# kianmcevoy/audio_analysis

Measured on AMD Instinct MI355X. Metric: IRs/sec full report (STFT+RT60bands+zplane), 48 kHz 10 s IR, higher is better.
Workload: dtype f64; 1 GPU; metrics-only full report on 256 mono synthetic IRs per GPU per step, 10 s @ 48 kHz (SURVEY.md 8d generator), H2D included: every step uploads its batch from pinned host memory (float32, 492 MB) on a copy stream under the previous step's kernels; 4 distinct batches rotate; batch_per_gpu=256, parallelism=file-sharded dp1, gather=final

## Files before the change

audio_analysis_amd/_lib.py:

```python
from __future__ import annotations

import ctypes as C
from pathlib import Path

_LIB_PATH = Path(__file__).resolve().parent / "csrc" / "libira.so"
_lib = None
ABI_VERSION = 15

c_f32p = C.c_void_p
c_i64p = C.c_void_p
c_i32p = C.c_void_p
c_f64p = C.c_void_p
vp = C.c_void_p
i32 = C.c_int32
f64 = C.c_double
f32 = C.c_float

PROTOTYPES = {
    "ira_abi_version": (i32, []),
    "ira_error_string": (C.c_char_p, [i32]),
    "ira_peak_index": (i32, [vp, vp, vp, i32, C.c_int64, vp, vp, vp]),
    "ira_edc_db": (i32, [vp, vp, vp, i32, C.c_int64, f64, f64, vp, vp, vp, vp, vp]),
    "ira_curve_fits": (i32, [vp, vp, vp, i32, i32, f32, f32, vp, C.POINTER(f64), i32, i32, C.POINTER(f64), i32, i32,
                             f64, f64, vp, vp, vp]),
# ... 18 lines not shown
    "ira_band_tile_layout": (i32, [i32, i32, C.POINTER(i32), C.POINTER(i32)]),
    "ira_wav_probe": (i32, [C.c_char_p, vp, vp, vp, vp]),
    "ira_wav_read_pcm16": (i32, [C.c_char_p, C.c_int64, C.c_int64, i32, vp]),
    "ira_wav_probe_batch": (i32, [vp, i32, i32, vp, vp, vp, vp, vp]),
    "ira_wav_read_pcm16_batch": (i32, [vp, vp, vp, vp, vp, vp, i32, i32, vp]),
    "ira_pcm16_to_channels": (i32, [vp, C.c_int64, i32, i32, vp, vp]),
    "ira_pcm16_to_channels_jobs": (i32, [vp, vp, vp, vp, vp, vp, i32, C.c_int64, vp, vp]),
    "ira_band_mask_values": (i32, [C.POINTER(f64), f64, C.c_int64, vp, vp]),
    "ira_host_pull": (i32, [vp, C.c_int64, i32, vp, i32, vp]),
    "ira_deconv_divide": (i32, [vp, vp, vp, vp, vp, i32, i32, f64, vp, vp]),
    "ira_deconv_finish": (i32, [vp, vp, vp, vp, i32, i32, i32, i32, i32, f64, vp, vp, vp]),
    "ira_order_stats": (i32, [vp, vp, vp, i32, vp, i32, vp, vp]),
    "ira_diffusion": (i32, [vp, vp, vp, i32, i32, i32, i32, i32, f64, f64, vp, vp, vp, vp]),
    "ira_diffusion_stereo": (i32, [vp, vp, vp, vp, i32, i32, i32, i32, i32, vp, vp, vp, vp]),
    "ira_spectrum_stats": (i32, [vp, vp, vp, i32, vp, f64, f64, f64, vp, vp]),
    "ira_waterfall_rel": (i32, [vp, vp, vp, i32, i32, i32, i32, f64, vp, vp, vp]),
    "ira_logbin_aggregate": (i32, [vp, vp, vp, i32, i32, i32, vp, vp, i32, vp, vp, i32, vp]),
    "ira_ar_partial_doubles": (C.c_int64, [i32, i32]),
    "ira_ar_gram": (i32, [vp, vp, vp, vp, vp, i32, i32, i32, vp, i32, vp]),
    "ira_ar_solve": (i32, [vp, vp, i32, i32, i32, f64, vp, vp, vp, i32, vp]),
    "ira_ar_minnorm": (i32, [vp, vp, i32, i32, i32, vp, vp, vp, f64, vp]),
    "ira_ar_exact_doubles": (C.c_int64, [i32, i32, i32]),
    "ira_ar_exact": (i32, [vp, vp, vp, vp, vp, i32, i32, i32, f64, vp, vp, vp, vp, vp, f64, vp]),
    "ira_ar_refine": (i32, [vp, vp, vp, vp, vp, i32, i32, i32, vp, vp, vp, vp, vp, f64, i32, i32, vp]),
    "ira_ar_fit": (i32, [vp, vp, vp, vp, vp, i32, i32, i32, f64, vp, vp, vp, vp, i32, vp]),
    "ira_poly_roots": (i32, [vp, i32, i32, f64, vp, vp, vp]),
    "ira_fir_numerator": (i32, [vp, i32, vp, vp, vp, vp, i32, i32, vp, vp]),
    "ira_onset_index": (i32, [vp, vp, vp, i32, C.c_int64, vp, vp, f64, vp, vp]),
    "ira_energy_scratch_doubles": (C.c_int64, [i32, C.c_int64, i32]),
    "ira_energy_windows": (i32, [vp, vp, vp, vp, vp, i32, C.c_int64, vp, i32, vp, vp, vp]),
# ... 72 lines not shown
```

audio_analysis_amd/analyse/frequency_response.py:

```python
from __future__ import annotations

from dataclasses import dataclass
from pathlib import Path
from typing import List, Optional, Sequence, Tuple

import numpy as np

from ..engine import get_engine
from ._common import segment_bounds, segment_bounds_batch, wav_channels


@dataclass(frozen=True)
class FrequencyResponseAnalysisSettings:
    use_mono_downmix_for_stereo: bool = False
    trim_to_peak: bool = True
    ignore_leading_seconds: float = 0.0
    analysis_duration_seconds: Optional[float] = None
    use_hann_window: bool = True
    magnitude_floor_db: float = -120.0
    f_min_hz: float = 20.0
    f_max_hz: float = 20000.0
    smoothing_log_bins: int = 0
    log_bins_per_octave: int = 96

# ... 62 lines not shown


def spectrum_segments(eng, batch, sample_rate_hz: int, settings, what: str):
    peaks = eng.peaks(batch) if settings.trim_to_peak else np.zeros(batch.count, dtype=np.int64)
    starts, lens = segment_bounds_batch(batch.length, peaks, sample_rate_hz, settings.trim_to_peak,
                                        settings.ignore_leading_seconds, settings.analysis_duration_seconds)
    if np.any(lens < 32):
        raise ValueError(f"Not enough samples after trimming/selection to analyse {what}.")
    return starts, lens


def spectrum_device(eng, batch, sample_rate_hz: int, settings, what: str, want_phase: bool = False,
                    unwrap: bool = True, degrees: bool = True):
    starts, lens = spectrum_segments(eng, batch, sample_rate_hz, settings, what)
    spec, off, packed = eng.rfft_any_packed(batch.x, batch.off + starts, lens, bool(settings.use_hann_window))
    mag, ph = eng.spectrum_mag_phase(spec, off, lens, float(settings.magnitude_floor_db), want_phase=want_phase,
                                     packed=packed)
    phase = eng.phase_unwrap(ph, off, lens, unwrap, degrees) if want_phase else None
    nyq = 0.5 * float(sample_rate_hz)
    f_lo = float(np.clip(settings.f_min_hz, 0.0, nyq))
    f_hi = float(np.clip(settings.f_max_hz, f_lo, nyq))
    steps = np.array([rfft_bin_step(int(n), sample_rate_hz) for n in lens], dtype=np.float64)
    smoothed = False
    bins_w = int(getattr(settings, "smoothing_log_bins", 0) or 0)
    if bins_w > 1:
        s_lo = float(np.clip(settings.f_min_hz, 1.0, nyq))
        s_hi = float(np.clip(settings.f_max_hz, s_lo, nyq))
        rng = [selected_bin_range(int(n) // 2 + 1, float(st), max(1.0, s_lo), max(max(1.0, s_lo), s_hi))
               for n, st in zip(lens, steps)]
        k_lo = np.array([r[0] for r in rng], dtype=np.int32)
        nsel = np.array([r[1] for r in rng], dtype=np.int32)
        if np.all(nsel > 0):
            smoothed = eng.log_smooth(mag, off, np.ones(len(rng), np.int32), k_lo, nsel, steps, bins_w,
                                      int(getattr(settings, "log_bins_per_octave", 96)), through_float32=False)
    stats = eng.spectrum_stats(mag, off, lens, steps, f_lo, f_hi, 1000.0)
    return dict(spec=spec if packed is None else None, spec_packed=spec if packed is not None else None, off=off, packed=packed, starts=starts, lens=lens, mag=mag, phase=phase, stats=stats, f_lo=f_lo,
                f_hi=f_hi, smoothed=smoothed)


def analyse_frequency_response_batch(
    channels: Sequence[np.ndarray],
    sample_rate_hz: int,
    channel_names: Sequence[str],
    settings: FrequencyResponseAnalysisSettings,
) -> List[ChannelFrequencyResponse]:
    for c in channels:
        if c.ndim != 1:
            raise ValueError("analyse_frequency_response_for_channel expects a 1D mono array.")
    eng = get_engine()
    batch = eng.upload(list(channels))
# ... 103 lines not shown
```

audio_analysis_amd/analyse/group_delay.py:

```python
from __future__ import annotations

from dataclasses import dataclass
from pathlib import Path
from typing import List, Optional, Sequence, Tuple

import numpy as np

from ..engine import get_engine
from ._common import wav_channels
from .frequency_response import rfft_bin_step


@dataclass(frozen=True)
class GroupDelayAnalysisSettings:
    use_mono_downmix_for_stereo: bool = False
    trim_to_peak: bool = True
    ignore_leading_seconds: float = 0.0
    analysis_duration_seconds: Optional[float] = None
    use_hann_window: bool = True
    fft_size: Optional[int] = None
    f_min_hz: float = 20.0
    f_max_hz: float = 20000.0
    unwrap_phase: bool = True
    smoothing_bins: int = 0
# ... 48 lines not shown
    n = batch.count
    if starts is None:
        peaks = eng.peaks(batch) if settings.trim_to_peak else np.zeros(n, dtype=np.int64)
        starts = np.empty(n, dtype=np.int64)
        lens = np.empty(n, dtype=np.int64)
        for i in range(n):
            starts[i], lens[i] = group_delay_segment(int(batch.length[i]), int(peaks[i]), sample_rate_hz, settings)
    if np.any(lens < 1):
        raise ValueError("Not enough samples after trimming/selection to analyse group delay.")
    n_fft = np.array([fft_size_for(int(v), settings) for v in lens], dtype=np.int64)
    if np.any(n_fft < 2) or np.any(n_fft > (1 << 21)):
        raise ValueError("group delay needs 2 <= fft_size <= 2097152.")
    with eng.tagged("[gd]"):
        spec, off = eng.rfft_any(batch.x, batch.off + starts, n_fft.astype(np.int32), bool(settings.use_hann_window),
                                 data_len=np.minimum(lens, n_fft).astype(np.int32), win_len=lens.astype(np.int32))
        _, ph = eng.spectrum_mag_phase(spec, off, n_fft.astype(np.int32), -400.0, want_phase=True)
        ph64 = eng.phase_unwrap(ph, off, n_fft.astype(np.int32), bool(settings.unwrap_phase), False, as_float64=True)
        steps = np.array([rfft_bin_step(int(v), sample_rate_hz) for v in n_fft], dtype=np.float64)
        gd = eng.group_delay(ph64, off, n_fft, steps, float(sample_rate_hz))
    return dict(gd=gd, off=off, n_fft=n_fft, starts=starts, lens=lens)


_MASK_CACHE: dict = {}


def mask_range(n_fft: int, sample_rate_hz: int, f_min_hz: float, f_max_hz: float) -> Tuple[int, int]:
    key = (int(n_fft), int(sample_rate_hz), float(f_min_hz), float(f_max_hz))
    if key not in _MASK_CACHE:
        freq = np.fft.rfftfreq(int(n_fft), d=1.0 / float(sample_rate_hz))
        idx = np.nonzero((freq >= float(f_min_hz)) & (freq <= float(f_max_hz)))[0]
        _MASK_CACHE[key] = (int(idx[0]), int(idx.size)) if idx.size else (0, 0)
    return _MASK_CACHE[key]
# ... 146 lines not shown
```

audio_analysis_amd/csrc/ira_spectrum.hip:

```cpp
#include <cmath>

#include "ira_fft_reg.h"
#include "ira_log.h"

namespace {

typedef ira::cplx<double> cd;
constexpr double kPi = 3.14159265358979323846;

constexpr int ATAN_TAB = 64;

__device__ __forceinline__ void build_atan_table(double* tab, int tid) {
  if (tid <= ATAN_TAB) tab[tid] = atan((double)tid * (1.0 / ATAN_TAB));
}

__device__ __forceinline__ double atan2_table(double y, double x, const double* tab) {
  const double ax = fabs(x), ay = fabs(y);
  const double mx = fmax(ax, ay), mn = fmin(ax, ay);
  if (!(ax > 1.0e-300 && ay > 1.0e-300 && ax < 1.0e300 && ay < 1.0e300)) return atan2(y, x);
  const double t = mn / mx;
  const int k = (int)(t * (double)ATAN_TAB + 0.5);
  const double t0 = (double)k * (1.0 / ATAN_TAB);
  const double r = (t - t0) / fma(t, t0, 1.0);
  const double r2 = r * r;
  double s = fma(r2, 1.0 / 9.0, -1.0 / 7.0);
  s = fma(r2, s, 0.2);
  s = fma(r2, s, -1.0 / 3.0);
  s = fma(r2, s, 1.0);
  double a = fma(r, s, tab[k]);
  if (ay > ax) a = 1.5707963267948966 - a;
  if (x < 0.0) a = kPi - a;
  return copysign(a, y);
}

__device__ __forceinline__ double unwrap_correction(double prev, double cur) {
  const double dd = cur - prev;
  const double period = 2.0 * kPi;
  double a = dd + kPi;
  double md;
  if (a >= 0.0 && a < period) md = a;
  else if (a >= period && a < 2.0 * period) md = a - period;
  else if (a < 0.0 && a > -period) md = a;
  else md = fmod(a, period);
  if (md != 0.0) {
    if (md < 0.0) md += period;
  } else {
    md = 0.0;
  }
  double ddmod = md + (-kPi);
  if (ddmod == -kPi && dd > 0.0) ddmod = kPi;
  double corr = ddmod - dd;
  if (fabs(dd) < kPi) corr = 0.0;
  return corr;
}

__global__ __launch_bounds__(256) void mag_phase_kernel(const cd* __restrict__ spec, const int64_t* __restrict__ spec_off,
                                 const int32_t* __restrict__ L, double floor_lin, float* __restrict__ mag_db,
                                 const int64_t* __restrict__ mag_off, double* __restrict__ phase,
                                 const int64_t* __restrict__ phase_off, const int32_t* __restrict__ packed) {
  __shared__ ira::LogTabEntry ltab[ira::LOGTAB_N];
  __shared__ double atab[ATAN_TAB + 1];
  ira::build_log_table(ltab, threadIdx.x);
  build_atan_table(atab, threadIdx.x);
  __syncthreads();
  const int e = blockIdx.y;
  const long long nb = (long long)L[e] / 2 + 1;
  const cd* s = spec + spec_off[e];
  float* mo = mag_db + mag_off[e];
  double* po = phase ? phase + phase_off[e] : nullptr;
  const double floor_p = floor_lin * floor_lin;
  const float floor_db32 = (float)(20.0 * log10(floor_lin));
  const bool pk = packed != nullptr && ira::uniform(packed[e]) != 0;
  const long long l = (long long)L[e] / 2;
  const long long k_first = (long long)blockIdx.x * blockDim.x + threadIdx.x, k_step = (long long)gridDim.x * blockDim.x;
  double cs = 1.0, sn = 0.0, rc = 1.0, rs = 0.0;
  if (pk) {
    sincospi(-(double)(k_first < nb ? k_first : 0) / (double)l, &sn, &cs);
    sincospi(-(double)(k_step % (2 * l)) / (double)l, &rs, &rc);
  }
  for (long long k = k_first; k < nb; k += k_step) {
    cd v;
    if (pk) {
      const cd zk = s[k == l ? 0 : k], zl = s[(k == 0 || k == l) ? 0 : l - k];
      const auto [ev, od] = ira::hermitian_parts(zk, zl);
      v = {ev.re + (cs * od.re - sn * od.im), ev.im + (cs * od.im + sn * od.re)};
      if (k == 0 || k == l) v.im = 0.0;
      const double nc = cs * rc - sn * rs;
      sn = sn * rc + cs * rs;
      cs = nc;
    } else {
      v = s[k];
    }
    const double p = v.re * v.re + v.im * v.im;
    float db;
    if (p > 1.0e-280 && p < 1.0e280 && floor_lin > 1.0e-140) {
      db = p > floor_p ? (float)(3.0102999566398120 * ira::log2_table(p, ltab)) : floor_db32;
    } else {
      const double a = hypot(v.re, v.im);
      const double m = (a != a) ? a : fmax(a, floor_lin);
      db = (float)(20.0 * log10(m));
    }
    mo[k] = db;
    if (po) po[k] = atan2_table(v.im, v.re, atab);
  }
}

constexpr int UW_THREADS = 1024;
constexpr int UW_PER = 4;
constexpr int UW_TILE = UW_THREADS * UW_PER;

__global__ __launch_bounds__(UW_THREADS) void unwrap_kernel(const double* __restrict__ phase,
                                                            const int64_t* __restrict__ phase_off,
                                                            const int32_t* __restrict__ L, int do_unwrap,
                                                            double out_scale, float* __restrict__ out,
                                                            const int64_t* __restrict__ out_off,
                                                            double* __restrict__ out64) {
  __shared__ double wave_tot[UW_THREADS / IRA_WAVE];
  __shared__ double tile_total;
  const int e = blockIdx.x;
  const long long n = (long long)L[e] / 2 + 1;
  const double* p = phase + phase_off[e];
  float* o = out ? out + out_off[e] : nullptr;
  double* o64 = out64 ? out64 + out_off[e] : nullptr;
  const int t = threadIdx.x, lane = t & 63, wave = t >> 6;
// ... 11 lines not shown
    double prev = nprev;
#pragma unroll
    for (int r = 0; r < UW_PER; ++r) v[r] = nv[r];
    if (base + UW_TILE < n) {
      const long long j0 = i0 + UW_TILE;
      nprev = (j0 - 1 < n) ? p[j0 - 1] : 0.0;
#pragma unroll
      for (int r = 0; r < UW_PER; ++r) nv[r] = (j0 + r < n) ? p[j0 + r] : 0.0;
    }
#pragma unroll
    for (int r = 0; r < UW_PER; ++r) {
      const long long i = i0 + r;
      c[r] = (do_unwrap && i >= 1 && i < n) ? unwrap_correction(prev, v[r]) : 0.0;
      prev = v[r];
    }
    c[1] += c[0]; c[2] += c[1]; c[3] += c[2];
    double incl = c[3];
#pragma unroll
    for (int o2 = 1; o2 < 64; o2 <<= 1) {
      const double dn = __shfl_up(incl, o2, 64);
      if (lane >= o2) incl += dn;
    }
    double excl = __shfl_up(incl, 1, 64);
    if (lane == 0) excl = 0.0;
    if (lane == 63) wave_tot[wave] = incl;
    __syncthreads();
    double before = 0.0;
    for (int w = 0; w < wave; ++w) before += wave_tot[w];
    const double add = carry + (before + excl);
#pragma unroll
    for (int r = 0; r < UW_PER; ++r) {
      const long long i = i0 + r;
      if (i < n) {
        const double u = v[r] + (c[r] + add);
        if (o) o[i] = (float)(u * out_scale);
        if (o64) o64[i] = u;
      }
    }
    if (t == UW_THREADS - 1) tile_total = c[3] + add;
    __syncthreads();
    carry = tile_total;
  }
}

// ... 209 lines not shown
        const long long excl = incl - c;
        if ((excl <= rem && rem < incl) || (tid == 255 && rem >= incl)) {
          remaining[r] = rem - excl;
          bucket[r] = c;
          prefix[r] = prefix[r] | ((unsigned long long)tid << shift);
        }
      }
      __syncthreads();
    }
  }
  if (tid < nranks) o[tid] = os_unkey(prefix[tid]);
}

constexpr int ST_THREADS = 1024;

__global__ __launch_bounds__(ST_THREADS) void stats_kernel(const float* __restrict__ mag_db,
                                                           const int64_t* __restrict__ mag_off,
                                                           const int32_t* __restrict__ L,
                                                           const double* __restrict__ freq_val, float f_min, float f_max,
                                                           float probe_hz, double* __restrict__ out) {
  __shared__ double red[4][ST_THREADS / IRA_WAVE];
  __shared__ unsigned long long kred[2][ST_THREADS / IRA_WAVE];
  __shared__ long long lred[ST_THREADS / IRA_WAVE];
  __shared__ double etab[ira::EXPTAB_N];
  const int e = blockIdx.x;
  const long long n = (long long)L[e] / 2 + 1;
  const float* m = mag_db + mag_off[e];
  const double val = freq_val[e];
  const int t = threadIdx.x, lane = t & 63, wave = t >> 6;
  ira::build_exp_table(etab, t);
  __syncthreads();
  double cnt = 0.0, sfl = 0.0, sl = 0.0;
  unsigned long long best = 0ull;
  unsigned long long near = ~0ull;
  long long first_in = n;
  constexpr int ST_U = 16;
  for (long long k0 = t; k0 < n; k0 += (long long)ST_THREADS * ST_U) {
    float dbv[ST_U];
#pragma unroll
    for (int u = 0; u < ST_U; ++u) {
      const long long k = k0 + (long long)ST_THREADS * u;
      dbv[u] = m[k < n ? k : n - 1];
    }
#pragma unroll
    for (int u = 0; u < ST_U; ++u) {
      const long long k = k0 + (long long)ST_THREADS * u;
      if (k >= n) continue;
      const float f = (float)((double)k * val);
      const float d = fabsf(f - probe_hz);
      const unsigned long long nk = ((unsigned long long)__float_as_uint(d) << 32) | (unsigned long long)(uint32_t)k;
      near = nk < near ? nk : near;
      if (f >= f_min && f <= f_max) {
        const float db = dbv[u];
        uint32_t uu = __float_as_uint(db);
        uu = (uu & 0x80000000u) ? ~uu : (uu | 0x80000000u);
        if (db != db) uu = 0xFFFFFFFFu;
        const unsigned long long key = ((unsigned long long)uu << 32) | (unsigned long long)(0xFFFFFFFFu - (uint32_t)k);
        best = key > best ? key : best;
        const double y = (double)db * 0.05;
        const double lin = fabs(y) < 15.0 ? ira::exp10_table(y, etab) : exp10(y);
        cnt += 1.0; sfl += (double)f * lin; sl += lin;
        first_in = k < first_in ? k : first_in;
      }
    }
  }
  cnt = ira::wave_sum(cnt); sfl = ira::wave_sum(sfl); sl = ira::wave_sum(sl);
#pragma unroll
  for (int o = 32; o > 0; o >>= 1) {
    const unsigned long long ob = __shfl_xor(best, o, 64);
    best = ob > best ? ob : best;
    const unsigned long long on = __shfl_xor(near, o, 64);
    near = on < near ? on : near;
    const long long of = __shfl_xor(first_in, o, 64);
    first_in = of < first_in ? of : first_in;
  }
  if (lane == 0) {
    red[0][wave] = cnt; red[1][wave] = sfl; red[2][wave] = sl;
    kred[0][wave] = best; kred[1][wave] = near; lred[wave] = first_in;
  }
  __syncthreads();
  if (t == 0) {
    cnt = sfl = sl = 0.0;
    for (int w = 0; w < ST_THREADS / IRA_WAVE; ++w) {
      cnt += red[0][w]; sfl += red[1][w]; sl += red[2][w];
      best = kred[0][w] > best ? kred[0][w] : best;
      near = kred[1][w] < near ? kred[1][w] : near;
      first_in = lred[w] < first_in ? lred[w] : first_in;
    }
    double* o = out + (int64_t)e * 8;
    const long long pk = (cnt > 0.0) ? (long long)(0xFFFFFFFFu - (uint32_t)(best & 0xFFFFFFFFull)) : 0;
    const long long i1k = (long long)(near & 0xFFFFFFFFull);
    o[0] = cnt;
    o[1] = (double)pk;
    o[2] = (double)(float)((double)pk * val);
    o[3] = sfl; o[4] = sl;
    o[5] = first_in < n ? (double)(float)((double)first_in * val) : 0.0;
    o[6] = (double)i1k;
    o[7] = (double)m[i1k];
  }
}

constexpr int LS_MAX = 2048;
constexpr int LS_THREADS = 256;

__device__ __forceinline__ double ls_freq(long long k, double fstep) { return (double)(float)((double)k * fstep); }

__global__ __launch_bounds__(LS_THREADS) void log_smooth_kernel(float* __restrict__ mag, const int64_t* __restrict__ off,
                                                                const int32_t* __restrict__ stride_a,
                                                                const int32_t* __restrict__ k_lo_a,
                                                                const int32_t* __restrict__ nsel_a,
                                                                const double* __restrict__ fstep_a,
                                                                const double* __restrict__ lg_lo, const double* __restrict__ lg_hi,
                                                                const int32_t* __restrict__ count_a, int window,
                                                                int through_f32) {
// ... 106 lines not shown
                                           gd_dev);
  IRA_RETURN_LAUNCH();
}

extern "C" int32_t ira_spectrum_stats(const float* mag_db_dev, const int64_t* mag_off_dev, const int32_t* L_dev,
                                      int32_t nb, const double* freq_val_dev, double f_min_hz, double f_max_hz,
                                      double probe_hz, double* out_dev, void* stream) {
  IRA_CHECK_PTR(mag_db_dev); IRA_CHECK_PTR(mag_off_dev); IRA_CHECK_PTR(L_dev); IRA_CHECK_PTR(freq_val_dev);
  IRA_CHECK_PTR(out_dev);
  if (nb <= 0) return nb == 0 ? IRA_OK : IRA_E_SIZE;
  stats_kernel<<<nb, ST_THREADS, 0, (hipStream_t)stream>>>(mag_db_dev, mag_off_dev, L_dev, freq_val_dev,
                                                           (float)f_min_hz, (float)f_max_hz, (float)probe_hz, out_dev);
  IRA_RETURN_LAUNCH();
}

extern "C" int32_t ira_order_stats(const double* values_dev, const int64_t* off_dev, const int32_t* count_dev,
                                   int32_t nseg, const int64_t* ranks_dev, int32_t nranks, double* out_dev,
                                   void* stream) {
  IRA_CHECK_PTR(values_dev); IRA_CHECK_PTR(off_dev); IRA_CHECK_PTR(count_dev); IRA_CHECK_PTR(ranks_dev);
  IRA_CHECK_PTR(out_dev);
  if (nranks < 1 || nranks > OS_MAX_RANKS) return IRA_E_SIZE;
  if (nseg <= 0) return nseg == 0 ? IRA_OK : IRA_E_SIZE;
  order_stats_kernel<<<nseg, OS_THREADS, 0, (hipStream_t)stream>>>(values_dev, off_dev, count_dev, ranks_dev, nranks,
                                                                    out_dev);
  IRA_RETURN_LAUNCH();
}

extern "C" int32_t ira_log_smooth_db(float* mag_dev, const int64_t* off_dev, const int32_t* stride_dev,
                                     const int32_t* k_lo_dev, const int32_t* nsel_dev, const double* fstep_dev,
                                     const double* log2_lo_dev, const double* log2_hi_dev, const int32_t* count_dev,
// ... 13 lines not shown
```

audio_analysis_amd/engine.py:

```python
from __future__ import annotations

import ctypes
import math
import os
from contextlib import contextmanager
from dataclasses import dataclass, fields
from typing import Dict, List, Optional, Sequence, Tuple

import numpy as np

from . import _lib
from ._lib import IraError, check
from .engine_plan import (SMOOTH, Switches, conv_size, exclusive_cumsum, pair_bands, plan_band_irfft,
                          plan_rfft)

FIT_DOUBLES = 8
EDC_SCRATCH_DOUBLES = 4096
EDC_TILE = 4096


def _ptr(t) -> int:
    return 0 if t is None else int(t.data_ptr())


# ... 1090 lines not shown

    def spectrum_mag_phase(self, spec_dev, spec_off: np.ndarray, lengths: np.ndarray, floor_db: float,
                           want_phase: bool, packed: Optional[np.ndarray] = None):
        t = self.torch
        n = int(spec_off.size)
        lengths = np.ascontiguousarray(lengths, dtype=np.int32)
        total = int((lengths.astype(np.int64) // 2 + 1).sum())
        mag = self.empty(total, t.float32)
        ph = self.empty(total, t.float64) if want_phase else None
        d_so, d_l, d_pk = self.job_tables(spec_off, lengths, None if packed is None else np.ascontiguousarray(packed, np.int32))
        check(self.lib.ira_spectrum_mag_phase(_ptr(spec_dev), _ptr(d_so), _ptr(d_l), n, int(lengths.max()),
                                              float(floor_db), _ptr(mag), _ptr(d_so), _ptr(ph), _ptr(d_so), _ptr(d_pk),
                                              self.stream), "ira_spectrum_mag_phase")
        return mag, ph

    def phase_unwrap(self, phase_dev, off: np.ndarray, lengths: np.ndarray, unwrap: bool, degrees: bool,
                     as_float64: bool = False):
        t = self.torch
        lengths = np.ascontiguousarray(lengths, dtype=np.int32)
        total = int((lengths.astype(np.int64) // 2 + 1).sum())
        out = self.empty(total, t.float64 if as_float64 else t.float32)
        d_o, d_l = self.job_tables(off, lengths)
        check(self.lib.ira_phase_unwrap(_ptr(phase_dev), _ptr(d_o), _ptr(d_l), int(off.size), 1 if unwrap else 0,
                                        1 if degrees else 0, 0 if as_float64 else _ptr(out), _ptr(d_o),
                                        _ptr(out) if as_float64 else 0, self.stream), "ira_phase_unwrap")
        return out

    def log_smooth(self, mag_dev, off: np.ndarray, stride: np.ndarray, k_lo: np.ndarray, nsel: np.ndarray,
                   fstep: np.ndarray, window: int, bins_per_octave: int, through_float32: bool) -> bool:
        n = int(np.asarray(off).size)
# ... 212 lines not shown
```

include/ira.h:

```cpp
#ifndef IRA_H_
#define IRA_H_

#include <stdint.h>

#ifdef __cplusplus
extern "C" {
#endif

#define IRA_OK 0
#define IRA_E_NULL (-1)
#define IRA_E_SIZE (-2)
#define IRA_E_UNSUPPORTED (-3)
#define IRA_E_IO (-4)
#define IRA_E_FORMAT (-5)
#define IRA_E_HIP_BASE (-1000)

#define IRA_ABI_VERSION 15

int32_t ira_abi_version(void);
const char* ira_error_string(int32_t code);

int32_t ira_peak_index(const float* x_dev, const int64_t* off_dev, const int64_t* len_dev,
                       int32_t nseg, int64_t max_len, int64_t* peak_dev, float* peak_abs_dev, void* stream);

// ... 67 lines not shown
                               int32_t nb, int32_t max_len, double floor_db, float* mag_db_dev,
                               const int64_t* mag_off_dev, double* phase_dev,
                               const int64_t* phase_off_dev, const int32_t* packed_dev, void* stream);

int32_t ira_phase_unwrap(const double* phase_dev, const int64_t* phase_off_dev, const int32_t* L_dev,
                         int32_t nb, int32_t do_unwrap, int32_t to_degrees, float* out_dev,
                         const int64_t* out_off_dev, double* out64_dev, void* stream);

int32_t ira_group_delay(const double* phase_dev, const int64_t* off_dev, const int32_t* nbins_dev, int32_t nb,
                        int32_t max_bins, const double* bin_step_dev, double sample_rate_hz, int32_t* flags_dev,
                        int32_t flags_known, double* gd_dev, void* stream);

int32_t ira_spectrum_stats(const float* mag_db_dev, const int64_t* mag_off_dev, const int32_t* L_dev,
                           int32_t nb, const double* freq_val_dev, double f_min_hz, double f_max_hz,
                           double probe_hz, double* out_dev, void* stream);

int32_t ira_waterfall_rel(const float* mag_dev, const int64_t* mag_off_dev, const int32_t* nslices_dev,
                          int32_t nb, int32_t k_lo, int32_t nsel, int32_t slice_max, double dyn_db,
                          float* out_dev, const int64_t* out_off_dev, void* stream);

int32_t ira_logbin_aggregate(const float* mag_dev, const int64_t* mag_off_dev, const int32_t* nframes_dev,
                             int32_t nb, int32_t max_frames, int32_t k_base, const int32_t* first_dev,
                             const int32_t* count_dev, int32_t nbins, float* out_dev,
                             const int64_t* out_off_dev, int32_t frame_major_rows, void* stream);

int32_t ira_log_smooth_db(float* mag_dev, const int64_t* off_dev, const int32_t* stride_dev, const int32_t* k_lo_dev,
                          const int32_t* nsel_dev, const double* fstep_dev, const double* log2_lo_dev,
                          const double* log2_hi_dev, const int32_t* count_dev, int32_t ncurves, int32_t max_count,
                          int32_t window, int32_t through_float32, void* stream);

// ... 175 lines not shown
```

Measured before the change: 15410 IRs/s.

## Fuse spectrum magnitude, phase unwrap and stats into one finish kernel

Adds a spectrum_finish kernel that, per spectrum, unpacks the packed FFT bins, writes dB magnitude, computes phase with a tiled unwrap scan, and accumulates the spectrum statistics in one pass. Frequency response and group delay now call it instead of running separate mag/phase, unwrap and stats launches. This removes the intermediate phase array round-trip through memory and the re-read of the magnitudes for stats. In exchange the fused kernel is larger, uses more shared memory and runs one 1024-thread block per spectrum. Rare-path library calls are moved into noinline helpers to keep register use down.

```diff
diff --git a/audio_analysis_amd/_lib.py b/audio_analysis_amd/_lib.py
--- a/audio_analysis_amd/_lib.py
+++ b/audio_analysis_amd/_lib.py
@@ -56,6 +56,7 @@
     "ira_diffusion": (i32, [vp, vp, vp, i32, i32, i32, i32, i32, f64, f64, vp, vp, vp, vp]),
     "ira_diffusion_stereo": (i32, [vp, vp, vp, vp, i32, i32, i32, i32, i32, vp, vp, vp, vp]),
     "ira_spectrum_stats": (i32, [vp, vp, vp, i32, vp, f64, f64, f64, vp, vp]),
+    "ira_spectrum_finish": (i32, [vp, vp, vp, i32, f64, vp, vp, vp, i32, i32, vp, vp, vp, vp, f64, f64, f64, vp, vp]),
     "ira_waterfall_rel": (i32, [vp, vp, vp, i32, i32, i32, i32, f64, vp, vp, vp]),
     "ira_logbin_aggregate": (i32, [vp, vp, vp, i32, i32, i32, vp, vp, i32, vp, vp, i32, vp]),
     "ira_ar_partial_doubles": (C.c_int64, [i32, i32]),
diff --git a/audio_analysis_amd/analyse/frequency_response.py b/audio_analysis_amd/analyse/frequency_response.py
--- a/audio_analysis_amd/analyse/frequency_response.py
+++ b/audio_analysis_amd/analyse/frequency_response.py
@@ -100,15 +100,16 @@
                     unwrap: bool = True, degrees: bool = True):
     starts, lens = spectrum_segments(eng, batch, sample_rate_hz, settings, what)
     spec, off, packed = eng.rfft_any_packed(batch.x, batch.off + starts, lens, bool(settings.use_hann_window))
-    mag, ph = eng.spectrum_mag_phase(spec, off, lens, float(settings.magnitude_floor_db), want_phase=want_phase,
-                                     packed=packed)
-    phase = eng.phase_unwrap(ph, off, lens, unwrap, degrees) if want_phase else None
     nyq = 0.5 * float(sample_rate_hz)
     f_lo = float(np.clip(settings.f_min_hz, 0.0, nyq))
     f_hi = float(np.clip(settings.f_max_hz, f_lo, nyq))
     steps = np.array([rfft_bin_step(int(n), sample_rate_hz) for n in lens], dtype=np.float64)
     smoothed = False
     bins_w = int(getattr(settings, "smoothing_log_bins", 0) or 0)
+    done = eng.spectrum_finish(spec, off, lens, float(settings.magnitude_floor_db), packed=packed, want_phase=want_phase,
+                               unwrap=unwrap, degrees=degrees,
+                               stats=None if bins_w > 1 else (steps, f_lo, f_hi, 1000.0))
+    mag, phase, stats = done["mag"], done["phase"], done["stats"]
     if bins_w > 1:
         s_lo = float(np.clip(settings.f_min_hz, 1.0, nyq))
         s_hi = float(np.clip(settings.f_max_hz, s_lo, nyq))
@@ -119,7 +120,7 @@
         if np.all(nsel > 0):
             smoothed = eng.log_smooth(mag, off, np.ones(len(rng), np.int32), k_lo, nsel, steps, bins_w,
                                       int(getattr(settings, "log_bins_per_octave", 96)), through_float32=False)
-    stats = eng.spectrum_stats(mag, off, lens, steps, f_lo, f_hi, 1000.0)
+        stats = eng.spectrum_stats(mag, off, lens, steps, f_lo, f_hi, 1000.0)
     return dict(spec=spec if packed is None else None, spec_packed=spec if packed is not None else None, off=off, packed=packed, starts=starts, lens=lens, mag=mag, phase=phase, stats=stats, f_lo=f_lo,
                 f_hi=f_hi, smoothed=smoothed)
 
diff --git a/audio_analysis_amd/analyse/group_delay.py b/audio_analysis_amd/analyse/group_delay.py
--- a/audio_analysis_amd/analyse/group_delay.py
+++ b/audio_analysis_amd/analyse/group_delay.py
@@ -86,8 +86,8 @@
     with eng.tagged("[gd]"):
         spec, off = eng.rfft_any(batch.x, batch.off + starts, n_fft.astype(np.int32), bool(settings.use_hann_window),
                                  data_len=np.minimum(lens, n_fft).astype(np.int32), win_len=lens.astype(np.int32))
-        _, ph = eng.spectrum_mag_phase(spec, off, n_fft.astype(np.int32), -400.0, want_phase=True)
-        ph64 = eng.phase_unwrap(ph, off, n_fft.astype(np.int32), bool(settings.unwrap_phase), False, as_float64=True)
+        ph64 = eng.spectrum_finish(spec, off, n_fft.astype(np.int32), want_mag=False, want_phase=True,
+                                   unwrap=bool(settings.unwrap_phase), degrees=False, as_float64=True)["phase"]
         steps = np.array([rfft_bin_step(int(v), sample_rate_hz) for v in n_fft], dtype=np.float64)
         gd = eng.group_delay(ph64, off, n_fft, steps, float(sample_rate_hz))
     return dict(gd=gd, off=off, n_fft=n_fft, starts=starts, lens=lens)
diff --git a/audio_analysis_amd/csrc/ira_spectrum.hip b/audio_analysis_amd/csrc/ira_spectrum.hip
--- a/audio_analysis_amd/csrc/ira_spectrum.hip
+++ b/audio_analysis_amd/csrc/ira_spectrum.hip
@@ -9,6 +9,20 @@
 constexpr double kPi = 3.14159265358979323846;
 
 constexpr int ATAN_TAB = 64;
+
+__device__ __attribute__((noinline)) double atan2_lib(double y, double x) { return atan2(y, x); }
+__device__ __attribute__((noinline)) double fmod_lib(double a, double b) { return fmod(a, b); }
+__device__ __attribute__((noinline)) double exp10_lib(double y) { return exp10(y); }
+__device__ __attribute__((noinline)) cd twiddle_lib(long long k, long long l) {
+  double sn, cs;
+  sincospi(-(double)(k % (2 * l)) / (double)l, &sn, &cs);
+  return {cs, sn};
+}
+__device__ __attribute__((noinline)) float db_lib(double re, double im, double floor_lin) {
+  const double a = hypot(re, im);
+  const double m = (a != a) ? a : fmax(a, floor_lin);
+  return (float)(20.0 * log10(m));
+}
 
 __device__ __forceinline__ void build_atan_table(double* tab, int tid) {
   if (tid <= ATAN_TAB) tab[tid] = atan((double)tid * (1.0 / ATAN_TAB));
@@ -17,7 +31,7 @@
 __device__ __forceinline__ double atan2_table(double y, double x, const double* tab) {
   const double ax = fabs(x), ay = fabs(y);
   const double mx = fmax(ax, ay), mn = fmin(ax, ay);
-  if (!(ax > 1.0e-300 && ay > 1.0e-300 && ax < 1.0e300 && ay < 1.0e300)) return atan2(y, x);
+  if (!(ax > 1.0e-300 && ay > 1.0e-300 && ax < 1.0e300 && ay < 1.0e300)) return atan2_lib(y, x);
   const double t = mn / mx;
   const int k = (int)(t * (double)ATAN_TAB + 0.5);
   const double t0 = (double)k * (1.0 / ATAN_TAB);
@@ -41,7 +55,7 @@
   if (a >= 0.0 && a < period) md = a;
   else if (a >= period && a < 2.0 * period) md = a - period;
   else if (a < 0.0 && a > -period) md = a;
-  else md = fmod(a, period);
+  else md = fmod_lib(a, period);
   if (md != 0.0) {
     if (md < 0.0) md += period;
   } else {
@@ -52,6 +66,22 @@
   double corr = ddmod - dd;
   if (fabs(dd) < kPi) corr = 0.0;
   return corr;
+}
+
+__device__ __forceinline__ cd packed_bin(cd zk, cd zl, double cs, double sn, bool edge) {
+  const auto [ev, od] = ira::hermitian_parts(zk, zl);
+  cd v = {ev.re + (cs * od.re - sn * od.im), ev.im + (cs * od.im + sn * od.re)};
+  if (edge) v.im = 0.0;
+  return v;
+}
+
+__device__ __forceinline__ float bin_db(cd v, double floor_lin, double floor_p, float floor_db32,
+                                        const ira::LogTabEntry* ltab) {
+  const double p = v.re * v.re + v.im * v.im;
+  if (p > 1.0e-280 && p < 1.0e280 && floor_lin > 1.0e-140) {
+    return p > floor_p ? (float)(3.0102999566398120 * ira::log2_table(p, ltab)) : floor_db32;
+  }
+  return db_lib(v.re, v.im, floor_lin);
 }
 
 __global__ __launch_bounds__(256) void mag_phase_kernel(const cd* __restrict__ spec, const int64_t* __restrict__ spec_off,
@@ -81,26 +111,14 @@
   for (long long k = k_first; k < nb; k += k_step) {
     cd v;
     if (pk) {
-      const cd zk = s[k == l ? 0 : k], zl = s[(k == 0 || k == l) ? 0 : l - k];
-      const auto [ev, od] = ira::hermitian_parts(zk, zl);
-      v = {ev.re + (cs * od.re - sn * od.im), ev.im + (cs * od.im + sn * od.re)};
-      if (k == 0 || k == l) v.im = 0.0;
+      v = packed_bin(s[k == l ? 0 : k], s[(k == 0 || k == l) ? 0 : l - k], cs, sn, k == 0 || k == l);
       const double nc = cs * rc - sn * rs;
       sn = sn * rc + cs * rs;
       cs = nc;
     } else {
       v = s[k];
     }
-    const double p = v.re * v.re + v.im * v.im;
-    float db;
-    if (p > 1.0e-280 && p < 1.0e280 && floor_lin > 1.0e-140) {
-      db = p > floor_p ? (float)(3.0102999566398120 * ira::log2_table(p, ltab)) : floor_db32;
-    } else {
-      const double a = hypot(v.re, v.im);
-      const double m = (a != a) ? a : fmax(a, floor_lin);
-      db = (float)(20.0 * log10(m));
-    }
-    mo[k] = db;
+    mo[k] = bin_db(v, floor_lin, floor_p, floor_db32, ltab);
     if (po) po[k] = atan2_table(v.im, v.re, atab);
   }
 }
@@ -108,6 +126,23 @@
 constexpr int UW_THREADS = 1024;
 constexpr int UW_PER = 4;
 constexpr int UW_TILE = UW_THREADS * UW_PER;
+
+__device__ __forceinline__ double unwrap_scan(double (&c)[UW_PER], double carry, double* wave_tot, int lane, int wave) {
+  c[1] += c[0]; c[2] += c[1]; c[3] += c[2];
+  double incl = c[3];
+#pragma unroll
+  for (int o2 = 1; o2 < 64; o2 <<= 1) {
+    const double dn = __shfl_up(incl, o2, 64);
+    if (lane >= o2) incl += dn;
+  }
+  double excl = __shfl_up(incl, 1, 64);
+  if (lane == 0) excl = 0.0;
+  if (lane == 63) wave_tot[wave] = incl;
+  __syncthreads();
+  double before = 0.0;
+  for (int w = 0; w < wave; ++w) before += wave_tot[w];
+  return carry + (before + excl);
+}
 
 __global__ __launch_bounds__(UW_THREADS) void unwrap_kernel(const double* __restrict__ phase,
                                                             const int64_t* __restrict__ phase_off,
@@ -149,20 +184,7 @@
       c[r] = (do_unwrap && i >= 1 && i < n) ? unwrap_correction(prev, v[r]) : 0.0;
       prev = v[r];
     }
-    c[1] += c[0]; c[2] += c[1]; c[3] += c[2];
-    double incl = c[3];
-#pragma unroll
-    for (int o2 = 1; o2 < 64; o2 <<= 1) {
-      const double dn = __shfl_up(incl, o2, 64);
-      if (lane >= o2) incl += dn;
-    }
-    double excl = __shfl_up(incl, 1, 64);
-    if (lane == 0) excl = 0.0;
-    if (lane == 63) wave_tot[wave] = incl;
-    __syncthreads();
-    double before = 0.0;
-    for (int w = 0; w < wave; ++w) before += wave_tot[w];
-    const double add = carry + (before + excl);
+    const double add = unwrap_scan(c, carry, wave_tot, lane, wave);
 #pragma unroll
     for (int r = 0; r < UW_PER; ++r) {
       const long long i = i0 + r;
@@ -402,26 +424,95 @@
 
 constexpr int ST_THREADS = 1024;
 
+struct StatsAcc {
+  double cnt = 0.0, sfl = 0.0, sl = 0.0;
+  unsigned long long best = 0ull;
+  unsigned long long near = ~0ull;
+  long long first_in;
+  float near_db = 0.0f;
+};
+struct StatsScratch {
+  double red[3][ST_THREADS / IRA_WAVE];
+  unsigned long long kred[2][ST_THREADS / IRA_WAVE];
+  long long lred[ST_THREADS / IRA_WAVE];
+  float dred[ST_THREADS / IRA_WAVE];
+};
+
+__device__ __forceinline__ void stats_bin(StatsAcc& a, long long k, float db, double val, float f_min, float f_max,
+                                          float probe_hz, const double* etab) {
+  const float f = (float)((double)k * val);
+  const float d = fabsf(f - probe_hz);
+  const unsigned long long nk = ((unsigned long long)__float_as_uint(d) << 32) | (unsigned long long)(uint32_t)k;
+  a.near_db = nk < a.near ? db : a.near_db;
+  a.near = nk < a.near ? nk : a.near;
+  if (f >= f_min && f <= f_max) {
+    uint32_t uu = __float_as_uint(db);
+    uu = (uu & 0x80000000u) ? ~uu : (uu | 0x80000000u);
+    if (db != db) uu = 0xFFFFFFFFu;
+    const unsigned long long key = ((unsigned long long)uu << 32) | (unsigned long long)(0xFFFFFFFFu - (uint32_t)k);
+    a.best = key > a.best ? key : a.best;
+    const double y = (double)db * 0.05;
+    const double lin = fabs(y) < 15.0 ? ira::exp10_table(y, etab) : exp10_lib(y);
+    a.cnt += 1.0; a.sfl += (double)f * lin; a.sl += lin;
+    a.first_in = k < a.first_in ? k : a.first_in;
+  }
+}
+
+__device__ __forceinline__ void stats_finish(StatsAcc a, StatsScratch& sc, long long n, double val, double* o) {
+  const int t = threadIdx.x, lane = t & 63, wave = t >> 6;
+  a.cnt = ira::wave_sum(a.cnt); a.sfl = ira::wave_sum(a.sfl); a.sl = ira::wave_sum(a.sl);
+#pragma unroll
+  for (int o2 = 32; o2 > 0; o2 >>= 1) {
+    const unsigned long long ob = __shfl_xor(a.best, o2, 64);
+    a.best = ob > a.best ? ob : a.best;
+    const unsigned long long on = __shfl_xor(a.near, o2, 64);
+    const float od = __shfl_xor(a.near_db, o2, 64);
+    a.near_db = on < a.near ? od : a.near_db;
+    a.near = on < a.near ? on : a.near;
+    const long long of = __shfl_xor(a.first_in, o2, 64);
+    a.first_in = of < a.first_in ? of : a.first_in;
+  }
+  if (lane == 0) {
+    sc.red[0][wave] = a.cnt; sc.red[1][wave] = a.sfl; sc.red[2][wave] = a.sl;
+    sc.kred[0][wave] = a.best; sc.kred[1][wave] = a.near; sc.lred[wave] = a.first_in; sc.dred[wave] = a.near_db;
+  }
+  __syncthreads();
+  if (t == 0) {
+    a.cnt = a.sfl = a.sl = 0.0;
+    for (int w = 0; w < ST_THREADS / IRA_WAVE; ++w) {
+      a.cnt += sc.red[0][w]; a.sfl += sc.red[1][w]; a.sl += sc.red[2][w];
+      a.best = sc.kred[0][w] > a.best ? sc.kred[0][w] : a.best;
+      a.near_db = sc.kred[1][w] < a.near ? sc.dred[w] : a.near_db;
+      a.near = sc.kred[1][w] < a.near ? sc.kred[1][w] : a.near;
+      a.first_in = sc.lred[w] < a.first_in ? sc.lred[w] : a.first_in;
+    }
+    const long long pk = (a.cnt > 0.0) ? (long long)(0xFFFFFFFFu - (uint32_t)(a.best & 0xFFFFFFFFull)) : 0;
+    o[0] = a.cnt;
+    o[1] = (double)pk;
+    o[2] = (double)(float)((double)pk * val);
+    o[3] = a.sfl; o[4] = a.sl;
+    o[5] = a.first_in < n ? (double)(float)((double)a.first_in * val) : 0.0;
+    o[6] = (double)(long long)(a.near & 0xFFFFFFFFull);
+    o[7] = (double)a.near_db;
+  }
+}
+
 __global__ __launch_bounds__(ST_THREADS) void stats_kernel(const float* __restrict__ mag_db,
                                                            const int64_t* __restrict__ mag_off,
                                                            const int32_t* __restrict__ L,
                                                            const double* __restrict__ freq_val, float f_min, float f_max,
                                                            float probe_hz, double* __restrict__ out) {
-  __shared__ double red[4][ST_THREADS / IRA_WAVE];
-  __shared__ unsigned long long kred[2][ST_THREADS / IRA_WAVE];
-  __shared__ long long lred[ST_THREADS / IRA_WAVE];
+  __shared__ StatsScratch sc;
   __shared__ double etab[ira::EXPTAB_N];
   const int e = blockIdx.x;
   const long long n = (long long)L[e] / 2 + 1;
   const float* m = mag_db + mag_off[e];
   const double val = freq_val[e];
-  const int t = threadIdx.x, lane = t & 63, wave = t >> 6;
+  const int t = threadIdx.x;
   ira::build_exp_table(etab, t);
   __syncthreads();
-  double cnt = 0.0, sfl = 0.0, sl = 0.0;
-  unsigned long long best = 0ull;
-  unsigned long long near = ~0ull;
-  long long first_in = n;
+  StatsAcc acc;
+  acc.first_in = n;
   constexpr int ST_U = 16;
   for (long long k0 = t; k0 < n; k0 += (long long)ST_THREADS * ST_U) {
     float dbv[ST_U];
@@ -434,58 +525,145 @@
     for (int u = 0; u < ST_U; ++u) {
       const long long k = k0 + (long long)ST_THREADS * u;
       if (k >= n) continue;
-      const float f = (float)((double)k * val);
-      const float d = fabsf(f - probe_hz);
-      const unsigned long long nk = ((unsigned long long)__float_as_uint(d) << 32) | (unsigned long long)(uint32_t)k;
-      near = nk < near ? nk : near;
-      if (f >= f_min && f <= f_max) {
-        const float db = dbv[u];
-        uint32_t uu = __float_as_uint(db);
-        uu = (uu & 0x80000000u) ? ~uu : (uu | 0x80000000u);
-        if (db != db) uu = 0xFFFFFFFFu;
-        const unsigned long long key = ((unsigned long long)uu << 32) | (unsigned long long)(0xFFFFFFFFu - (uint32_t)k);
-        best = key > best ? key : best;
-        const double y = (double)db * 0.05;
-        const double lin = fabs(y) < 15.0 ? ira::exp10_table(y, etab) : exp10(y);
-        cnt += 1.0; sfl += (double)f * lin; sl += lin;
-        first_in = k < first_in ? k : first_in;
-      }
-    }
-  }
-  cnt = ira::wave_sum(cnt); sfl = ira::wave_sum(sfl); sl = ira::wave_sum(sl);
-#pragma unroll
-  for (int o = 32; o > 0; o >>= 1) {
-    const unsigned long long ob = __shfl_xor(best, o, 64);
-    best = ob > best ? ob : best;
-    const unsigned long long on = __shfl_xor(near, o, 64);
-    near = on < near ? on : near;
-    const long long of = __shfl_xor(first_in, o, 64);
-    first_in = of < first_in ? of : first_in;
-  }
-  if (lane == 0) {
-    red[0][wave] = cnt; red[1][wave] = sfl; red[2][wave] = sl;
-    kred[0][wave] = best; kred[1][wave] = near; lred[wave] = first_in;
-  }
+      stats_bin(acc, k, dbv[u], val, f_min, f_max, probe_hz, etab);
+    }
+  }
+  stats_finish(acc, sc, n, val, out + (int64_t)e * 8);
+}
+
+constexpr int SF_TWQ = 512;
+constexpr int SF_STAGE = 2;
+
+template <bool DB, bool PHASE>
+__global__ __launch_bounds__(UW_THREADS) void spectrum_finish_kernel(
+    const cd* __restrict__ spec, const int64_t* __restrict__ spec_off, const int32_t* __restrict__ L, double floor_lin,
+    const int32_t* __restrict__ packed, float* __restrict__ mag_db, const int64_t* __restrict__ out_off, int do_unwrap,
+    double out_scale, float* __restrict__ phase32, double* __restrict__ phase64, double* __restrict__ wrapped64,
+    const double* __restrict__ freq_val, float f_min, float f_max, float probe_hz, double* __restrict__ stats) {
+  static_assert(ST_THREADS == UW_THREADS, "the statistics' thread mapping is the tile's load mapping");
+  __shared__ ira::LogTabEntry ltab[ira::LOGTAB_N];
+  __shared__ double atab[ATAN_TAB + 1];
+  __shared__ double etab[ira::EXPTAB_N];
+  __shared__ StatsScratch sc;
+  __shared__ cd twq[SF_TWQ];
+  __shared__ double ph_tile[UW_TILE];
+  __shared__ double wave_tot[UW_THREADS / IRA_WAVE];
+  __shared__ double tile_total, prev_last;
+  const int e = blockIdx.x;
+  const int t = threadIdx.x, lane = t & 63, wave = t >> 6;
+  const long long len = ira::uniform(L[e]);
+  const long long n = len / 2 + 1, l = len / 2;
+  const cd* s = spec + ira::uniform(spec_off[e]);
+  const long long oo = ira::uniform(out_off[e]);
+  const bool pk = packed != nullptr && ira::uniform(packed[e]) != 0 && l > 0;
+  const bool want_stats = DB && stats != nullptr;
+  const double val = want_stats ? ira::uniform(freq_val[e]) : 0.0;
+  const double floor_p = floor_lin * floor_lin;
+  const float floor_db32 = (float)(20.0 * log10(floor_lin));
+  if constexpr (DB) ira::build_log_table(ltab, t);
+  if constexpr (PHASE) build_atan_table(atab, t);
+  if (want_stats) ira::build_exp_table(etab, t);
+  double wt_c = 1.0, wt_s = 0.0;
+  auto build_twq = [&](long long q0) {
+    const long long k = (q0 + t) * UW_THREADS;
+    if (t < SF_TWQ && k < n) twq[t] = twiddle_lib(k, l);
+  };
+  if (pk) {
+    const cd wt = twiddle_lib(t, l);
+    wt_c = wt.re;
+    wt_s = wt.im;
+    build_twq(0);
+  }
+  if (t == 0) { tile_total = 0.0; prev_last = 0.0; }
   __syncthreads();
-  if (t == 0) {
-    cnt = sfl = sl = 0.0;
-    for (int w = 0; w < ST_THREADS / IRA_WAVE; ++w) {
-      cnt += red[0][w]; sfl += red[1][w]; sl += red[2][w];
-      best = kred[0][w] > best ? kred[0][w] : best;
-      near = kred[1][w] < near ? kred[1][w] : near;
-      first_in = lred[w] < first_in ? lred[w] : first_in;
-    }
-    double* o = out + (int64_t)e * 8;
-    const long long pk = (cnt > 0.0) ? (long long)(0xFFFFFFFFu - (uint32_t)(best & 0xFFFFFFFFull)) : 0;
-    const long long i1k = (long long)(near & 0xFFFFFFFFull);
-    o[0] = cnt;
-    o[1] = (double)pk;
-    o[2] = (double)(float)((double)pk * val);
-    o[3] = sfl; o[4] = sl;
-    o[5] = first_in < n ? (double)(float)((double)first_in * val) : 0.0;
-    o[6] = (double)i1k;
-    o[7] = (double)m[i1k];
-  }
+  StatsAcc acc;
+  acc.first_in = n;
+  cd nza[SF_STAGE], nzb[SF_STAGE];
+  auto load_stage = [&](long long first) {
+#pragma unroll
+    for (int r = 0; r < SF_STAGE; ++r) {
+      const long long k = first + t + (long long)UW_THREADS * r;
+      nza[r] = {0.0, 0.0};
+      nzb[r] = {0.0, 0.0};
+      if (k < n) {
+        if (pk) {
+          nza[r] = s[k == l ? 0 : k];
+          nzb[r] = s[(k == 0 || k == l) ? 0 : l - k];
+        } else {
+          nza[r] = s[k];
+        }
+      }
+    }
+  };
+  load_stage(0);
+  for (long long base = 0; base < n; base += UW_TILE) {
+    if (pk && base > 0 && base % ((long long)SF_TWQ * UW_THREADS) == 0) {
+      __syncthreads();
+      build_twq(base / UW_THREADS);
+      __syncthreads();
+    }
+    const long long qb = base / ((long long)SF_TWQ * UW_THREADS) * SF_TWQ;
+#pragma unroll 1
+    for (int h = 0; h < UW_PER / SF_STAGE; ++h) {
+      const long long first = base + (long long)h * SF_STAGE * UW_THREADS;
+      cd za[SF_STAGE], zb[SF_STAGE];
+#pragma unroll
+      for (int r = 0; r < SF_STAGE; ++r) { za[r] = nza[r]; zb[r] = nzb[r]; }
+      if (first + SF_STAGE * UW_THREADS < n) load_stage(first + SF_STAGE * UW_THREADS);
+#pragma unroll
+      for (int r = 0; r < SF_STAGE; ++r) {
+        const int j = t + UW_THREADS * (h * SF_STAGE + r);
+        const long long k = base + j;
+        double ph = 0.0;
+        if (k < n) {
+          cd v = za[r];
+          if (pk) {
+            const cd w = twq[k / UW_THREADS - qb];
+            const double cs = w.re * wt_c - w.im * wt_s;
+            const double sn = w.im * wt_c + w.re * wt_s;
+            v = packed_bin(za[r], zb[r], cs, sn, k == 0 || k == l);
+          }
+          if constexpr (DB) {
+            const float db = bin_db(v, floor_lin, floor_p, floor_db32, ltab);
+            mag_db[oo + k] = db;
+            if (want_stats) stats_bin(acc, k, db, val, f_min, f_max, probe_hz, etab);
+          }
+          if constexpr (PHASE) {
+            ph = atan2_table(v.im, v.re, atab);
+            if (wrapped64) wrapped64[oo + k] = ph;
+          }
+        }
+        if constexpr (PHASE) ph_tile[j] = ph;
+      }
+    }
+    if constexpr (PHASE) {
+      __syncthreads();
+      const double carry = tile_total;
+      const long long i0 = base + (long long)UW_PER * t;
+      double c[UW_PER], v[UW_PER];
+      double prev = t == 0 ? prev_last : ph_tile[UW_PER * t - 1];
+#pragma unroll
+      for (int r = 0; r < UW_PER; ++r) v[r] = ph_tile[UW_PER * t + r];
+#pragma unroll
+      for (int r = 0; r < UW_PER; ++r) {
+        const long long i = i0 + r;
+        c[r] = (do_unwrap && i >= 1 && i < n) ? unwrap_correction(prev, v[r]) : 0.0;
+        prev = v[r];
+      }
+      const double add = unwrap_scan(c, carry, wave_tot, lane, wave);
+#pragma unroll
+      for (int r = 0; r < UW_PER; ++r) {
+        const long long i = i0 + r;
+        if (i < n) {
+          const double u = v[r] + (c[r] + add);
+          if (phase32) phase32[oo + i] = (float)(u * out_scale);
+          if (phase64) phase64[oo + i] = u;
+        }
+      }
+      if (t == UW_THREADS - 1) { tile_total = c[3] + add; prev_last = v[3]; }
+    }
+  }
+  if (want_stats) stats_finish(acc, sc, n, val, stats + (int64_t)e * 8);
 }
 
 constexpr int LS_MAX = 2048;
@@ -622,6 +800,29 @@
   IRA_RETURN_LAUNCH();
 }
 
+extern "C" int32_t ira_spectrum_finish(const double* spec_dev, const int64_t* spec_off_dev, const int32_t* L_dev,
+                                       int32_t nb, double floor_db, const int32_t* packed_dev, float* mag_db_dev,
+                                       const int64_t* out_off_dev, int32_t do_unwrap, int32_t to_degrees,
+                                       float* phase32_dev, double* phase64_dev, double* wrapped64_dev,
+                                       const double* freq_val_dev, double f_min_hz, double f_max_hz, double probe_hz,
+                                       double* stats_dev, void* stream) {
+  IRA_CHECK_PTR(spec_dev); IRA_CHECK_PTR(spec_off_dev); IRA_CHECK_PTR(L_dev); IRA_CHECK_PTR(out_off_dev);
+  const bool phase = phase32_dev != nullptr || phase64_dev != nullptr || wrapped64_dev != nullptr;
+  if (mag_db_dev == nullptr && !phase) return IRA_E_NULL;
+  if (stats_dev != nullptr && (mag_db_dev == nullptr || freq_val_dev == nullptr)) return IRA_E_NULL;
+  if (nb <= 0) return nb == 0 ? IRA_OK : IRA_E_SIZE;
+  const double floor_lin = std::pow(10.0, floor_db / 20.0);
+  const double scale = to_degrees ? (180.0 / kPi) : 1.0;
+  auto kernel = spectrum_finish_kernel<true, true>;
+  if (!phase) kernel = spectrum_finish_kernel<true, false>;
+  if (mag_db_dev == nullptr) kernel = spectrum_finish_kernel<false, true>;
+  kernel<<<nb, UW_THREADS, 0, (hipStream_t)stream>>>(
+      reinterpret_cast<const cd*>(spec_dev), spec_off_dev, L_dev, floor_lin, packed_dev, mag_db_dev, out_off_dev,
+      do_unwrap ? 1 : 0, scale, phase32_dev, phase64_dev, wrapped64_dev, freq_val_dev, (float)f_min_hz, (float)f_max_hz,
+      (float)probe_hz, stats_dev);
+  IRA_RETURN_LAUNCH();
+}
+
 extern "C" int32_t ira_order_stats(const double* values_dev, const int64_t* off_dev, const int32_t* count_dev,
                                    int32_t nseg, const int64_t* ranks_dev, int32_t nranks, double* out_dev,
                                    void* stream) {
diff --git a/audio_analysis_amd/engine.py b/audio_analysis_amd/engine.py
--- a/audio_analysis_amd/engine.py
+++ b/audio_analysis_amd/engine.py
@@ -1128,6 +1128,29 @@
                                               self.stream), "ira_spectrum_mag_phase")
         return mag, ph
 
+    def spectrum_finish(self, spec_dev, off: np.ndarray, lengths: np.ndarray, floor_db: float = -120.0,
+                        packed: Optional[np.ndarray] = None, want_mag: bool = True, want_phase: bool = False,
+                        unwrap: bool = True, degrees: bool = True, as_float64: bool = False, want_wrapped: bool = False,
+                        stats: Optional[tuple] = None):
+        t = self.torch
+        n = int(off.size)
+        lengths = np.ascontiguousarray(lengths, dtype=np.int32)
+        total = int((lengths.astype(np.int64) // 2 + 1).sum())
+        mag = self.empty(total, t.float32) if want_mag else None
+        phase = self.empty(total, t.float64 if as_float64 else t.float32) if want_phase else None
+        wrapped = self.empty(total, t.float64) if want_wrapped else None
+        rec = self.empty(n * 8, t.float64) if stats is not None else None
+        freq_val, f_min, f_max, probe_hz = stats if stats is not None else (None, 0.0, 0.0, 0.0)
+        d_o, d_l, d_pk, d_fv = self.job_tables(off, lengths,
+                                               None if packed is None else np.ascontiguousarray(packed, np.int32),
+                                               None if freq_val is None else np.ascontiguousarray(freq_val, np.float64))
+        check(self.lib.ira_spectrum_finish(_ptr(spec_dev), _ptr(d_o), _ptr(d_l), n, float(floor_db), _ptr(d_pk), _ptr(mag),
+                                           _ptr(d_o), 1 if unwrap else 0, 1 if degrees else 0,
+                                           0 if as_float64 else _ptr(phase), _ptr(phase) if as_float64 else 0,
+                                           _ptr(wrapped), _ptr(d_fv), float(f_min), float(f_max), float(probe_hz),
+                                           _ptr(rec), self.stream), "ira_spectrum_finish")
+        return dict(mag=mag, phase=phase, wrapped=wrapped, stats=None if rec is None else rec[: n * 8].view(n, 8))
+
     def phase_unwrap(self, phase_dev, off: np.ndarray, lengths: np.ndarray, unwrap: bool, degrees: bool,
                      as_float64: bool = False):
         t = self.torch
diff --git a/include/ira.h b/include/ira.h
--- a/include/ira.h
+++ b/include/ira.h
@@ -105,6 +105,12 @@
 int32_t ira_spectrum_stats(const float* mag_db_dev, const int64_t* mag_off_dev, const int32_t* L_dev,
                            int32_t nb, const double* freq_val_dev, double f_min_hz, double f_max_hz,
                            double probe_hz, double* out_dev, void* stream);
+
+int32_t ira_spectrum_finish(const double* spec_dev, const int64_t* spec_off_dev, const int32_t* L_dev, int32_t nb,
+                            double floor_db, const int32_t* packed_dev, float* mag_db_dev, const int64_t* out_off_dev,
+                            int32_t do_unwrap, int32_t to_degrees, float* phase32_dev, double* phase64_dev,
+                            double* wrapped64_dev, const double* freq_val_dev, double f_min_hz, double f_max_hz,
+                            double probe_hz, double* stats_dev, void* stream);
 
 int32_t ira_waterfall_rel(const float* mag_dev, const int64_t* mag_off_dev, const int32_t* nslices_dev,
                           int32_t nb, int32_t k_lo, int32_t nsel, int32_t slice_max, double dyn_db,
```

Result: faster. 15610 IRs/s (median of 6 runs) (+1.3%).
